# davidea97/Fisher-Nerf-customized

Hardware: AMD Instinct MI355X
Metric: candidate-views/sec (higher is better)
Workload: dtype f32

## Files before the change

### fisher-nerf-customized_amd/csrc/fisher_rast.hip

```cpp
#include <hip/hip_runtime.h>
#include <hip/hip_fp16.h>
#include <stdint.h>
#include <stdio.h>
#include <stdlib.h>
#include <string.h>
#include "fr_math.h"
#include "../../include/fisher_rast.h"
#include "fr_internal.h"

#define FR_THREADS 256
#define FR_G_MAX 32
#define FR_MAX_LDS_TILES 4096
#define FR_PART_MIN_DEFAULT 2048
#define FR_SORT_SMALL_KEYS 2048
#define FR_SORT_MID_KEYS 4096
#define FR_SORT_BIG_KEYS 16384
#define FR_VC_MAX 16
#define FR_BATCH 256
#define FR_BWD_BATCH 128

#include <vector>
#include <utility>
static thread_local char g_err[512] = "";
#if defined(FR_ABLATE) || defined(FR_LOOPSTATS)
// ... 474 lines not shown
	}
	constexpr int NB = 8;
	for (int g0 = 0; g0 < p.G; g0 += NB)
	{
		int rad[NB];
		float4 q0[NB];
		float dep[NB];
#pragma unroll
		for (int b = 0; b < NB; b++)
		{
			const int i = (blockIdx.x * p.G + g0 + b) * FR_THREADS + tid;
			rad[b] = (g0 + b < p.G && i < p.P) ? p.radii[vP + i] : 0;
		}
#pragma unroll
		for (int b = 0; b < NB; b++)
		{
			const int i = (blockIdx.x * p.G + g0 + b) * FR_THREADS + tid;
			if (rad[b] > 0)
			{
				const float4* sp = (const float4*)(p.splat + vP + i);
				q0[b] = sp[0];
				dep[b] = sp[1].z;
			}
		}
#pragma unroll
		for (int b = 0; b < NB; b++)
		{
			if (rad[b] > 0)
			{
				const int i = (blockIdx.x * p.G + g0 + b) * FR_THREADS + tid;
				const uint64_t hi = ((uint64_t)fr_as_u32(dep[b])) << 32;
				const fr_rect rc = fr_get_rect(q0[b].x, q0[b].y, rad[b], p.gx, p.gy);
				for (uint32_t y = rc.y0; y < rc.y1; y++)
					for (uint32_t x = rc.x0; x < rc.x1; x++)
					{
						const uint32_t t = y * p.gx + x;
						const uint32_t slot = lds ? (s_base[t] + atomicAdd(&s_cnt[t], 1u)) : (off[t] + atomicAdd(&fill[t], 1u));
						p.keys[slot] = hi | (uint32_t)i;
					}
			}
		}
	}
}

struct FrRecordArgs {
	const float* H_inv; long long hinv_stride; const float* packed; float4* recq;
	const float4* mt;
	const float4* grp;
	int early;
	float4* comp;
	uint32_t* slot_idx;
	int stride;
	float* slot_acc;
};
template <int C> struct FrPackSize { static constexpr int value = (C >= 11) ? 32 : 16; };
template <int C, bool REWRITE, bool FORM_A = false, bool FIVE = false, bool IDV = false>
__device__ __forceinline__ void fr_fisher_record_one(const FrParams& p, const float* __restrict__ H_inv, long long hinv_stride,
                                                     const float* __restrict__ packed, float4* __restrict__ recq, int v, uint32_t id,
                                                     const float* vm, const float* pm, const float* wm, bool has_w2c,
                                                     float4* out6 = nullptr, const float4* ab_src = nullptr);
template <int C, int AF, bool DK = false> struct FrRecStride { static constexpr int value = AF == 4 ? 3 : AF >= 2 ? (C >= 11 ? 13 : 7) : ((AF == 0 && DK) ? 5 : 6); };
template <int C, bool POSE = false>
__device__ __forceinline__ void fr_fisher_record_general(const FrParams& p, const float* __restrict__ packed, int v, uint32_t id,
                                                         const float* vm, const float* pm, const float* wm, bool has_w2c,
                                                         float4* out, const float4* ab_src);

template <int RC, bool PHASE_C>
__global__ __launch_bounds__(FR_THREADS) void k_preprocess_views(FrParams p, FrRecordArgs ra)
{
	extern __shared__ uint32_t fr_dyn_lds[];
	const int VC = p.VC;
	uint32_t* hist = fr_dyn_lds;
	uint32_t* pairs = hist + (size_t)VC * p.T;
	float* s_wm = (float*)(pairs + FR_THREADS * VC);
	const int W32 = 8 * p.G;
	uint32_t* s_bm = (uint32_t*)(s_wm + 12 * VC);
	uint32_t* s_pf = s_bm + VC * W32;
	const bool compact = RC != 0 && ra.comp != nullptr;
	__shared__ uint32_t s_np;
	__shared__ uint32_t s_n[FR_VC_MAX];
	__shared__ uint32_t s_ref[FR_VC_MAX];
	const int tid = threadIdx.x, lane = tid & 63;
	const int v0 = blockIdx.y * VC;
	const int nv = min(VC, p.V - v0);
	const uint32_t nblk = gridDim.x;
	const uint32_t cap = (uint32_t)(FR_THREADS * p.G);
	for (int t = tid; t < nv * p.T; t += FR_THREADS) hist[t] = 0;
	const bool has_w2c = p.w2c != nullptr;
	if (has_w2c) for (int t = tid; t < nv * 12; t += FR_THREADS) s_wm[t] = p.w2c[16 * (size_t)(v0 + t / 12) + (t % 12)];
	if (tid < FR_VC_MAX) { s_n[tid] = 0; s_ref[tid] = 0; }
	if (tid == 0) s_np = 0;
	if (compact) for (int t = tid; t < nv * W32; t += FR_THREADS) s_bm[t] = 0u;
	float vm[16], pm[16];
#pragma unroll
	for (int k = 0; k < 16; k++) { vm[k] = p.view[k]; pm[k] = p.proj[k]; }
	__syncthreads();
	for (int g = 0; g < p.G; g++)
	{
		const int i0 = (blockIdx.x * p.G + g) * FR_THREADS;
		if (i0 >= p.P) break;
		{
			const int i = i0 + tid;
			const bool live = i < p.P;
			fr_f3 pw = { 0.f, 0.f, 0.f };
			if (live) pw = fr_f3{ p.means3D[3 * (size_t)i], p.means3D[3 * (size_t)i + 1], p.means3D[3 * (size_t)i + 2] };
			const bool early = RC != 0 && ra.early != 0 && ra.mt != nullptr;
			float tr = 0.f;
// ... 137 lines not shown
		if (p.vis_count && s_n[tid]) atomicAdd(&p.vis_count[v], (int)s_n[tid]);
		if (p.num_rendered && s_ref[tid]) atomicAdd(&p.num_rendered[v], (int)s_ref[tid]);
	}
	if constexpr (RC != 0 && PHASE_C)
	{
		__syncthreads();
		if (compact)
		{
			for (int t = tid; t < nv * W32; t += FR_THREADS)
			{
				const int vv = t / W32, w = t - vv * W32;
				uint32_t acc = 0;
				for (int u = 0; u < w; u++) acc += (uint32_t)__popc(s_bm[vv * W32 + u]);
				s_pf[t] = acc;
			}
			__syncthreads();
		}
		const size_t PV = (size_t)nblk * cap;
		for (int vv = 0; vv < nv; vv++)
		{
			const int v = v0 + vv;
			const uint32_t n = s_n[vv];
			FrVisEntry* list = p.vis_list + ((size_t)v * nblk + blockIdx.x) * cap;
			float wm[12];
#pragma unroll
			for (int k = 0; k < 12; k++) wm[k] = has_w2c ? s_wm[12 * vv + k] : 0.f;
			for (uint32_t e = tid; e < n; e += FR_THREADS)
			{
				const uint32_t idx = list[e].idx;
				if (compact)
				{
					const uint32_t local = idx - blockIdx.x * cap;
					const uint32_t rank = s_pf[vv * W32 + (int)(local >> 5)] + (uint32_t)__popc(s_bm[vv * W32 + (int)(local >> 5)] & ((1u << (local & 31u)) - 1u));
					const uint32_t slot = blockIdx.x * cap + rank;
					const float4* tmp = (const float4*)(p.splat + ((size_t)v * nblk + blockIdx.x) * cap + e);
					fr_fisher_record_one<(RC < 0 ? -RC : RC), false, (RC < 0)>(p, ra.H_inv, ra.hinv_stride, ra.packed, ra.recq, v, idx, vm, pm, wm, has_w2c,
					                                                           ra.comp + ((size_t)v * PV + slot) * 6, tmp);
					list[e].idx = slot;
					if constexpr (RC < 0) ra.slot_idx[(size_t)v * PV + slot] = idx;
				}
				else fr_fisher_record_one<(RC < 0 ? -RC : RC), false, (RC < 0)>(p, ra.H_inv, ra.hinv_stride, ra.packed, ra.recq, v, idx, vm, pm, wm, has_w2c);
			}
		}
	}
}

template <int C, int AF, bool DK, bool IDV = false, bool SLOTS = false>
__global__ __launch_bounds__(FR_THREADS) void k_preprocess_views_c(FrParams p, FrRecordArgs ra)
{
	static_assert(!SLOTS || (AF == 0 && !IDV), "the slot table is an option of the general score form (the out_H forms always write it)");
	static_assert((C == 4 || C == 11) && AF >= 0 && AF <= 4 && !((AF == 1 || AF >= 3) && C != 4), "records modes: score form, A-form (4 columns), general out_H form, pose form (4 columns), render form (4 columns)");
	static_assert(!IDV || (C == 4 && AF == 0 && DK), "the identity-view front end is the 4-column score form's with fixed key segments");
	constexpr int RS = FrRecStride<C, AF, DK>::value;
	extern __shared__ uint32_t fr_dyn_lds[];
	const int VC = p.VC;
	uint32_t* hist = fr_dyn_lds;
	uint32_t* pairs = hist + (size_t)VC * p.T;
	float* s_wm = (float*)(pairs + FR_THREADS * (VC + 1));
	uint32_t* park = (uint32_t*)(s_wm + 12 * VC);
	__shared__ uint32_t s_n[FR_VC_MAX];
	__shared__ uint32_t s_ref[FR_VC_MAX];
	__shared__ uint32_t s_ca[FR_VC_MAX * 4];
	__shared__ uint32_t s_wk2[2][FR_VC_MAX * 4];
	__shared__ uint32_t s_wtot2[2][4];
	uint32_t batch_no = 0;
	const int tid = threadIdx.x, lane = tid & 63;
	const int wave = __builtin_amdgcn_readfirstlane(tid >> 6);
	const int v0 = blockIdx.y * VC;
	const int nv = min(VC, p.V - v0);
	const uint32_t nblk = gridDim.x;
	const uint32_t cap = (uint32_t)(FR_THREADS * p.G);
	for (int t = tid; t < nv * p.T; t += FR_THREADS) hist[t] = 0;
	const bool has_w2c = p.w2c != nullptr;
	if (has_w2c) for (int t = tid; t < nv * 12; t += FR_THREADS) s_wm[t] = p.w2c[16 * (size_t)(v0 + t / 12) + (t % 12)];
	if (tid < FR_VC_MAX) { s_n[tid] = 0; s_ref[tid] = 0; }
	float vm[16], pm[16];
#pragma unroll
	for (int k = 0; k < 16; k++) { vm[k] = IDV ? (k % 5 == 0 ? 1.f : 0.f) : p.view[k]; pm[k] = p.proj[k]; }
	if constexpr (IDV)
	{
		bool id = true;
#pragma unroll
		for (int k = 0; k < 16; k++) id = id && p.view[k] == vm[k];
		if (!id && tid == 0) { atomicOr(&p.status[1], 1); atomicOr(&p.status[3], 2); }
	}
	const size_t PV = (size_t)nblk * cap;
	const unsigned long long lt = (1ull << lane) - 1ull;
	__syncthreads();
	const int iw = blockIdx.x * p.G * FR_THREADS;
	const bool early = ra.early != 0;
	const float lx = 1.3f * p.tanfovx, ly = 1.3f * p.tanfovy;
	float wn;
	{
		const float c0 = fabsf(vm[0]) + fabsf(vm[1]) + fabsf(vm[2]), c1 = fabsf(vm[4]) + fabsf(vm[5]) + fabsf(vm[6]), c2 = fabsf(vm[8]) + fabsf(vm[9]) + fabsf(vm[10]);
		const float r0 = fabsf(vm[0]) + fabsf(vm[4]) + fabsf(vm[8]), r1 = fabsf(vm[1]) + fabsf(vm[5]) + fabsf(vm[9]), r2 = fabsf(vm[2]) + fabsf(vm[6]) + fabsf(vm[10]);
		wn = fmaxf(c0, fmaxf(c1, c2)) * fmaxf(r0, fmaxf(r1, r2));
	}
	const float fx2 = 1.02f * wn * p.focal_x * p.focal_x, fy2 = 1.02f * wn * p.focal_y * p.focal_y;
	const float xmax = (float)(p.gx * FR_BLOCK_X + FR_BLOCK_X), ymax = (float)(p.gy * FR_BLOCK_Y + FR_BLOCK_Y);
	unsigned long long skipm = 0ull;
	if (early && ra.grp != nullptr && p.G * nv <= 64)
	{
		const float wrow = fabsf(pm[3] - vm[2]) + fabsf(pm[7] - vm[6]) + fabsf(pm[11] - vm[10]) + fabsf(pm[15] - vm[14]);
		const float wmag = fabsf(vm[2]) + fabsf(vm[6]) + fabsf(vm[10]) + fabsf(vm[14]);
		const bool pinhole = wrow <= 1e-6f * wmag;
		bool skip = false;
		const int g = lane / nv, vv = lane - g * nv;
		const int blk = blockIdx.x * p.G + g;
		if (pinhole && g < p.G && blk * FR_THREADS < p.P)
		{
#pragma clang fp contract(fast)
			const float4 b0 = ra.grp[2 * (size_t)blk], b1 = ra.grp[2 * (size_t)blk + 1];
			const fr_f3 cw = { 0.5f * (b0.x + b1.x), 0.5f * (b0.y + b1.y), 0.5f * (b0.z + b1.z) };
			const float ex = b1.x - cw.x, ey = b1.y - cw.y, ez = b1.z - cw.z;
			float R = 1.01f * __builtin_amdgcn_sqrtf(ex * ex + ey * ey + ez * ez) + 1e-6f;
			const fr_f3 c = has_w2c ? fr_world_to_cam(cw, s_wm + 12 * vv) : cw;
			if (has_w2c)
			{
				const float* m = s_wm + 12 * vv;
				const float g00 = m[0] * m[0] + m[4] * m[4] + m[8] * m[8], g11 = m[1] * m[1] + m[5] * m[5] + m[9] * m[9], g22 = m[2] * m[2] + m[6] * m[6] + m[10] * m[10];
				const float g01 = fabsf(m[0] * m[1] + m[4] * m[5] + m[8] * m[9]), g02 = fabsf(m[0] * m[2] + m[4] * m[6] + m[8] * m[10]), g12 = fabsf(m[1] * m[2] + m[5] * m[6] + m[9] * m[10]);
				R *= __builtin_amdgcn_sqrtf(fmaxf(g00 + g01 + g02, fmaxf(g01 + g11 + g12, g02 + g12 + g22))) * 1.00001f;
			}
			const float kcm = fx2 * (1.0f + lx * lx) + fy2 * (1.0f + ly * ly);
			const float a2 = 2.0f * 1.01f * 3.0f * __builtin_amdgcn_sqrtf(kcm * b0.w);
			const float c0 = 6.0f;
			const float Wf = (float)p.W, Hf = (float)p.H;
			const float zc = vm[2] * c.x + vm[6] * c.y + vm[10] * c.z + vm[14];
			const float zn = __builtin_amdgcn_sqrtf(vm[2] * vm[2] + vm[6] * vm[6] + vm[10] * vm[10]);
			auto side = [&](float sx, float sy, float sz, float sw, float kz, float add) -> bool {
				const float Ax = sx + kz * vm[2], Ay = sy + kz * vm[6], Az = sz + kz * vm[10];
				const float Lc = Ax * c.x + Ay * c.y + Az * c.z + (sw + kz * vm[14]) + add;
				return Lc + __builtin_amdgcn_sqrtf(Ax * Ax + Ay * Ay + Az * Az) * R < 0.f;
			};
			const bool left = side(Wf * pm[0], Wf * pm[4], Wf * pm[8], Wf * pm[12], Wf - 1.0f + 2.0f * c0, a2);
			const bool right = side(-Wf * pm[0], -Wf * pm[4], -Wf * pm[8], -Wf * pm[12], -(Wf - 1.0f - 2.0f * xmax - 2.0f * c0), a2);
			const bool top = side(Hf * pm[1], Hf * pm[5], Hf * pm[9], Hf * pm[13], Hf - 1.0f + 2.0f * c0, a2);
			const bool bottom = side(-Hf * pm[1], -Hf * pm[5], -Hf * pm[9], -Hf * pm[13], -(Hf - 1.0f - 2.0f * ymax - 2.0f * c0), a2);
			const bool behind = zc + zn * R <= 0.001f;
			skip = left || right || top || bottom || behind;
		}
		skipm = __builtin_amdgcn_ballot_w64(skip);
	}
	uint32_t pend = 0;
	for (int g = 0; g < p.G; g++)
	{
		const int i0 = iw + g * FR_THREADS;
		if (i0 >= p.P) break;
		const bool last_round = g == p.G - 1 || i0 + FR_THREADS >= p.P;
		uint32_t np = 0;
		const uint32_t skipv = (uint32_t)(skipm >> (g * nv)) & ((1u << nv) - 1u);
		if (skipv != (1u << nv) - 1u)
		{
			const int i = i0 + tid;
			const bool live = i < p.P;
			fr_f3 pw = { 0.f, 0.f, 0.f };
			float tr = 0.f;
			if (live) { const float4 m4 = ra.mt[i]; pw = fr_f3{ m4.x, m4.y, m4.z }; tr = m4.w; }
			uint32_t keepbits = 0;
			for (int vv = 0; vv < nv; vv++)
			{
// ... 128 lines not shown
					{
						const int tx0 = (int)ceilf((sp.px - hx - 15.0f) * 0.0625f), sy0 = (int)ceilf((sp.py - hy - 3.0f) * 0.25f);
						const int sy1 = (int)floorf((sp.py + hy) * 0.25f) + 1;
						rx0 = (uint32_t)max((int)rx0, tx0); rx1 = max(rx0, rx1);
						ry0 = (uint32_t)max((int)ry0, sy0); ry1 = (uint32_t)max((int)ry0, min((int)ry1, sy1));
					}
					if (rx1 > rx0 && ry1 > ry0)
						for (uint32_t y = ry0 >> 2; y <= (ry1 - 1u) >> 2; y++)
							for (uint32_t x = rx0; x < rx1; x++)
								atomicAdd(&h[y * p.gx + x], 1u);
				}
				else
				for (uint32_t y = ry0; y < ry1; y++)
					for (uint32_t x = rx0; x < rx1; x++)
						atomicAdd(&h[y * p.gx + x], 1u);
				park[0 * FR_THREADS + pos] = __float_as_uint(sp.px);
				park[1 * FR_THREADS + pos] = __float_as_uint(sp.py);
				park[2 * FR_THREADS + pos] = ext;
				if constexpr (AF == 4)
				{
					park[3 * FR_THREADS + pos] = __float_as_uint(o);
					park[4 * FR_THREADS + pos] = __float_as_uint(sp.conx);
					park[5 * FR_THREADS + pos] = __float_as_uint(sp.cony);
					park[6 * FR_THREADS + pos] = __float_as_uint(sp.conz);
				}
				else
				{
					park[3 * FR_THREADS + pos] = __float_as_uint(__builtin_amdgcn_logf(o));
					park[4 * FR_THREADS + pos] = __float_as_uint(-0.5f * sp.conx);
					park[5 * FR_THREADS + pos] = __float_as_uint(-sp.cony);
					park[6 * FR_THREADS + pos] = __float_as_uint(-0.5f * sp.conz);
				}
				park[7 * FR_THREADS + pos] = __float_as_uint(cg);
				park[8 * FR_THREADS + pos] = (uint32_t)i;
				park[9 * FR_THREADS + pos] = fr_as_u32(sp.depth);
				park[10 * FR_THREADS + pos] = rx0 | (ry0 << 16);
				park[11 * FR_THREADS + pos] = rx1 | (ry1 << 16);
				park[12 * FR_THREADS + pos] = rank | ((uint32_t)vv << 16);
			}
			__syncthreads();
			if (tid < nv) s_n[tid] += (s_wk[tid * 4] + s_wk[tid * 4 + 1]) + (s_wk[tid * 4 + 2] + s_wk[tid * 4 + 3]);
			FR_ABL(if (p.ablate == 36) nvis = 0;)
			if ((uint32_t)tid < nvis)
			{
					const int r = tid;
				float4 ab[2];
				ab[0] = make_float4(__uint_as_float(park[0 * FR_THREADS + r]), __uint_as_float(park[1 * FR_THREADS + r]),
				                    __uint_as_float(park[2 * FR_THREADS + r]), __uint_as_float(park[3 * FR_THREADS + r]));
				ab[1] = make_float4(__uint_as_float(park[4 * FR_THREADS + r]), __uint_as_float(park[5 * FR_THREADS + r]),
				                    __uint_as_float(park[6 * FR_THREADS + r]), __uint_as_float(park[7 * FR_THREADS + r]));
				const uint32_t idx = park[8 * FR_THREADS + r];
				const uint32_t rk = park[12 * FR_THREADS + r];
				const int cvv = (int)(rk >> 16);
				const uint32_t slot = blockIdx.x * cap + (rk & 0xffffu);
				const int v = v0 + cvv;
				float wm[12];
#pragma unroll
				for (int k = 0; k < 12; k++) wm[k] = has_w2c ? s_wm[12 * cvv + k] : 0.f;
				float4* rec_out = ra.comp + ((size_t)v * PV + slot) * RS;
				FR_ABL(if (p.ablate == 37) rec_out = ra.comp + (size_t)tid * RS;)
				if constexpr (AF == 4)
				{
					const float4 t2 = ((const float4*)(ra.packed + (size_t)idx * FrPackSize<C>::value))[2];
					rec_out[0] = ab[0];
					rec_out[1] = make_float4(ab[1].x, ab[1].y, ab[1].z, __uint_as_float(park[9 * FR_THREADS + r]));
					rec_out[2] = make_float4(t2.y, t2.z, t2.w, ab[1].w);
				}
				else if constexpr (AF >= 2) fr_fisher_record_general<C, (AF == 3)>(p, ra.packed, v, idx, vm, pm, wm, has_w2c, rec_out, ab);
				else fr_fisher_record_one<C, false, (AF == 1), (AF == 0 && DK), IDV>(p, ra.H_inv, ra.hinv_stride, ra.packed, ra.recq, v, idx, vm, pm, wm, has_w2c, rec_out, ab);
				if constexpr (DK)
				{
					const uint32_t xy0 = park[10 * FR_THREADS + r], xy1 = park[11 * FR_THREADS + r];
					const uint32_t rect = (xy0 & 255u) | ((xy0 >> 16) << 8) | (((xy1 & 0xffffu) - (xy0 & 0xffffu)) << 16) | (((xy1 >> 16) - (xy0 >> 16)) << 24);
					((uint2*)p.vis_list)[((size_t)v * nblk + blockIdx.x) * cap + (rk & 0xffffu)] = make_uint2(park[9 * FR_THREADS + r], rect);
				}
				else
				{
					FrVisEntry en;
					en.idx = slot; en.depth_bits = park[9 * FR_THREADS + r];
					en.xy0 = park[10 * FR_THREADS + r]; en.xy1 = park[11 * FR_THREADS + r];
					*(uint4*)(p.vis_list + ((size_t)v * nblk + blockIdx.x) * cap + (rk & 0xffffu)) = *(const uint4*)&en;
				}
				if constexpr (AF == 1 || AF == 2 || SLOTS) ra.slot_idx[(size_t)v * PV + slot] = p.order ? p.order[idx] : idx;
				if constexpr (SLOTS) ra.slot_acc[(size_t)v * PV + slot] = 0.f;
			}
		}
		const uint32_t rem = pend - ndo;
		if (rem != 0u && ndo != 0u)
		{
			uint32_t t = 0;
			if ((uint32_t)tid < rem) t = pairs[ndo + tid];
			__syncthreads();
			if ((uint32_t)tid < rem) pairs[tid] = t;
			__syncthreads();
		}
		pend = rem;
	}
	__syncthreads();
	if constexpr (DK)
	{
		uint32_t* cursor = park + 13 * FR_THREADS;
		uint32_t vend[FR_VC_MAX];
		uint32_t ntot = 0;
#pragma unroll
		for (int k = 0; k < FR_VC_MAX; k++) { if (k < nv) ntot += s_n[k]; vend[k] = ntot; }
		FR_ABL(if (p.ablate == 31) ntot = 0;)
		constexpr int NB = 4;
		uint2 en[NB], nx[NB];
		uint32_t ev[NB], nxv[NB];
		auto load_round = [&](uint32_t e0, uint2 (&de)[NB], uint32_t (&dv)[NB])
		{
#pragma unroll
			for (int b = 0; b < NB; b++)
			{
				const uint32_t e = e0 + b * FR_THREADS + tid;
				uint32_t vv = 0, lo = 0;
#pragma unroll
				for (int k = 0; k < FR_VC_MAX - 1; k++) if (e >= vend[k]) { vv = k + 1; lo = vend[k]; }
				dv[b] = vv;
				de[b] = make_uint2(0u, 0u);
				FR_ABL(if (p.ablate == 33) { if (e < ntot) de[b] = make_uint2(e, (e & 7u) | ((e >> 3 & 15u) << 10) | (2u << 16) | (2u << 24)); } else)
				if (e < ntot) de[b] = ((const uint2*)p.vis_list)[((size_t)(v0 + vv) * nblk + blockIdx.x) * cap + (e - lo)];
			}
		};
		load_round(0u, en, ev);
		const int nb = nv * p.T;
		for (int b0 = 0; b0 < nb; b0 += 4 * FR_THREADS)
		{
			uint32_t c[4], at[4], gt[4];
#pragma unroll
			for (int k = 0; k < 4; k++)
			{
				const int b = b0 + k * FR_THREADS + tid;
				c[k] = b < nb ? hist[b] : 0u;
				gt[k] = (uint32_t)(v0 + b / p.T) * (uint32_t)p.T + (uint32_t)(b % p.T);
			}
#pragma unroll
			for (int k = 0; k < 4; k++)
			{
				at[k] = 0u;
				FR_ABL(if (p.ablate != 34))
				if (c[k]) at[k] = atomicAdd(&p.tile_cnt[gt[k]], c[k]);
			}
#pragma unroll
			for (int k = 0; k < 4; k++)
			{
				const int b = b0 + k * FR_THREADS + tid;
				if (b < nb)
				{
					hist[b] = (c[k] && at[k] + c[k] <= p.tile_cap) ? gt[k] * p.tile_cap + at[k] : 0xffffffffu;
					cursor[b] = 0u;
				}
			}
		}
		__syncthreads();
		for (uint32_t e0 = 0; e0 < ntot; e0 += NB * FR_THREADS)
		{
			const bool more = e0 + NB * FR_THREADS < ntot;
			if (more) load_round(e0 + NB * FR_THREADS, nx, nxv);
#pragma unroll
			for (int b = 0; b < NB; b++)
			{
				const uint32_t e = e0 + b * FR_THREADS + tid;
				const uint32_t lo = ev[b] ? vend[ev[b] - 1] : 0u;
				const uint64_t key = ((uint64_t)en[b].x << 32) | ((blockIdx.x * cap + (e - lo)) << 4);
				const uint32_t r = en[b].y;
				const uint32_t x0 = r & 255u, s0 = (r >> 8) & 255u, x1 = x0 + ((r >> 16) & 255u), s1 = s0 + (r >> 24);
				const uint32_t* hb = hist + (size_t)ev[b] * p.T;
				uint32_t* cu = cursor + (size_t)ev[b] * p.T;
				if (x1 > x0 && s1 > s0)
				for (uint32_t y = s0 >> 2; y <= (s1 - 1u) >> 2; y++)
				{
					const uint32_t a = max(s0, 4u * y) - 4u * y, z = min(s1, 4u * y + 4u) - 4u * y;
					const uint64_t ky = key | (uint64_t)(((1u << z) - 1u) & ~((1u << a) - 1u));
					for (uint32_t x = x0; x < x1; x++)
					{
						const uint32_t t = y * p.gx + x;
						const uint32_t base = hb[t];
						const uint32_t k = atomicAdd(&cu[t], 1u);
						FR_ABL(if (p.ablate != 32 && p.ablate != 33))
						if (base != 0xffffffffu) p.keys[base + k] = ky;
					}
				}
			}
			if (more)
			{
#pragma unroll
				for (int b = 0; b < NB; b++) { en[b] = nx[b]; ev[b] = nxv[b]; }
			}
		}
	}
	else
	{
		for (int vv = 0; vv < nv; vv++)
		{
			const int v = v0 + vv;
			uint32_t* cnt = p.tile_cnt + (size_t)v * p.T;
			const uint32_t* h = hist + (size_t)vv * p.T;
			for (int t = tid; t < p.T; t += FR_THREADS)
			{
				const uint32_t c = h[t];
				if (c) p.blk_base[((size_t)v * nblk + blockIdx.x) * p.T + t] = atomicAdd(&cnt[t], c);
			}
		}
	}
	if (tid < nv)
	{
		const int v = v0 + tid;
		p.vis_n[(size_t)v * nblk + blockIdx.x] = s_n[tid];
		if (p.vis_count && s_n[tid]) atomicAdd(&p.vis_count[v], (int)s_n[tid]);
		if (p.num_rendered && s_ref[tid]) atomicAdd(&p.num_rendered[v], (int)s_ref[tid]);
	}
}
__global__ __launch_bounds__(FR_THREADS) void k_scatter_vis(FrParams p)
{
	extern __shared__ uint32_t fr_dyn_lds[];
	uint32_t* s_cnt = fr_dyn_lds;
	uint32_t* s_base = fr_dyn_lds + p.T;
	if (p.status[1]) return;
	const int tid = threadIdx.x;
	const int v = blockIdx.y;
	const uint32_t nblk = gridDim.x;
	const uint32_t n = p.vis_n[(size_t)v * nblk + blockIdx.x];
	if (n == 0) return;
	const uint32_t* off = p.tile_off + (size_t)v * p.T;
	const uint32_t* bb = p.blk_base + ((size_t)v * nblk + blockIdx.x) * p.T;
	for (int t = tid; t < p.T; t += FR_THREADS) { s_cnt[t] = 0; s_base[t] = off[t] + bb[t]; }
	__syncthreads();
	const uint4* list = (const uint4*)(p.vis_list + ((size_t)v * nblk + blockIdx.x) * (size_t)(FR_THREADS * p.G));
	constexpr int NB = 4;
	for (uint32_t e0 = 0; e0 < n; e0 += NB * FR_THREADS)
	{
		uint4 en[NB];
#pragma unroll
		for (int b = 0; b < NB; b++)
		{
			const uint32_t e = e0 + b * FR_THREADS + tid;
			en[b] = e < n ? list[e] : make_uint4(0u, 0u, 0u, 0u);
		}
#pragma unroll
		for (int b = 0; b < NB; b++)
		{
			const uint64_t key = ((uint64_t)en[b].y << 32) | en[b].x;
			const uint32_t x0 = en[b].z & 0xffffu, y0 = en[b].z >> 16, x1 = en[b].w & 0xffffu, y1 = en[b].w >> 16;
			for (uint32_t y = y0; y < y1; y++)
				for (uint32_t x = x0; x < x1; x++)
				{
					const uint32_t t = y * p.gx + x;
					p.keys[s_base[t] + atomicAdd(&s_cnt[t], 1u)] = key;
				}
		}
	}
}

__device__ __forceinline__ void fr_tile_of_block(const FrParams& p, uint32_t& tile, int& v, uint32_t first = 0u)
{
	const uint32_t L = blockIdx.x - first;
	if ((p.V & 7) == 0)
	{
		const uint32_t xcd = L & 7u, q = L >> 3;
		v = (int)((q / (uint32_t)p.T) * 8u + xcd);
		if (p.view_perm) v = (int)p.view_perm[v];
		tile = q % (uint32_t)p.T;
	}
	else
	{
		v = (int)(L / (uint32_t)p.T);
		tile = L % (uint32_t)p.T;
	}
}

__device__ __forceinline__ void fr_cx(uint64_t& lo, uint64_t& hi)
{
	const uint64_t a = lo, b = hi;
	const bool sw = a > b;
	lo = sw ? b : a; hi = sw ? a : b;
}
template <typename KeyPtr>
__device__ __forceinline__ uint64_t fr_ldk(KeyPtr keys, uint32_t i, uint32_t n) { return i < n ? keys[i] : ~0ull; }
template <typename KeyPtr>
__device__ __forceinline__ void fr_stk(KeyPtr keys, uint32_t i, uint32_t n, uint64_t v) { if (i < n) keys[i] = v; }

template <typename KeyPtr>
__device__ __forceinline__ void fr_bitonic(KeyPtr keys, uint32_t n, int tid, const uint32_t FR_NT = FR_THREADS)
{
	uint32_t n_pad = 1;
	while (n_pad < n) n_pad <<= 1;
	if (n_pad < 2) return;
	for (uint32_t t = tid; t < (n_pad >> 1); t += FR_NT)
	{
		uint64_t a = fr_ldk(keys, 2 * t, n), b = fr_ldk(keys, 2 * t + 1, n);
		fr_cx(a, b);
		fr_stk(keys, 2 * t, n, a); fr_stk(keys, 2 * t + 1, n, b);
	}
	__syncthreads();
	const uint32_t groups = n_pad >> 2;
	for (uint32_t k = 4, lk = 2; k <= n_pad; k <<= 1, lk++)
	{
		{
			const uint32_t q = k >> 2, qm = q - 1u;
			for (uint32_t g = tid; g < groups; g += FR_NT)
			{
				const uint32_t base = (g >> (lk - 2)) << lk, r = g & qm;
				const uint32_t ia = base + r, ib = ia + q, id = base + k - 1u - r, ic = id - q;
				uint64_t a = fr_ldk(keys, ia, n), b = fr_ldk(keys, ib, n), c = fr_ldk(keys, ic, n), d = fr_ldk(keys, id, n);
				fr_cx(a, d); fr_cx(b, c);
				fr_cx(a, b); fr_cx(c, d);
				fr_stk(keys, ia, n, a); fr_stk(keys, ib, n, b); fr_stk(keys, ic, n, c); fr_stk(keys, id, n, d);
			}
			__syncthreads();
		}
		uint32_t j = k >> 3, lj = lk - 3;
		for (; j >= 2; j >>= 2, lj -= 2)
		{
			const uint32_t h = j >> 1, lh = lj - 1, hm = h - 1u;
			for (uint32_t g = tid; g < groups; g += FR_NT)
			{
				const uint32_t i0 = ((g >> lh) << (lh + 2)) + (g & hm);
				const uint32_t i1 = i0 + h, i2 = i0 + j, i3 = i2 + h;
				uint64_t a = fr_ldk(keys, i0, n), b = fr_ldk(keys, i1, n), c = fr_ldk(keys, i2, n), d = fr_ldk(keys, i3, n);
				fr_cx(a, c); fr_cx(b, d);
				fr_cx(a, b); fr_cx(c, d);
// ... 5110 lines not shown
struct FrScorerPlan { int columns; bool form_a; FrRecordArgs ra; bool skip_pack = false; bool general = false; bool pose = false; bool view_identity = false; bool render = false; bool point = false; };
template <int C> __global__ void k_pack_static(FrParams p, const float* __restrict__ H_inv, float* __restrict__ packed, float4* __restrict__ mt, float4* __restrict__ grp);
template <int C, bool LIST, bool FORM_A> __global__ void k_fisher_records(FrParams p, FrRecordArgs ra);

static int fr_bin_pipeline(FrParams& p, const fr_gaussians* g, hipStream_t s, const FrScorerPlan* plan = nullptr)
{
	int rc;
	const int P = p.P;
	{
		FrZeroer z;
		z.add(p.tile_cnt, (size_t)p.V * p.T * 4); z.add(p.status, 16); z.add(p.big_list, 64);
		if (p.part_list) z.add(p.part_list, 4);
		if (p.view_work) z.add(p.view_work, (size_t)p.V * 4);
		if (p.vis_count) z.add(p.vis_count, (size_t)p.V * 4);
		if (p.num_rendered && p.vis_list != nullptr && p.T <= FR_MAX_LDS_TILES) z.add(p.num_rendered, (size_t)p.V * 4);
		z.launch(s);
	}
	const bool multi = p.vis_list != nullptr && p.T <= FR_MAX_LDS_TILES;
	if (g->cov3D_precomp) p.cov3D = g->cov3D_precomp;
	else if (plan && multi) p.cov3D = nullptr;
	else
	{
		hipLaunchKernelGGL(k_cov3d, dim3((P + FR_THREADS - 1) / FR_THREADS), dim3(FR_THREADS), 0, s, P, g->scales, p.mod, g->rotations, p.cov3D_out);
		if ((rc = fr_check_launch("k_cov3d"))) return rc;
		p.cov3D = p.cov3D_out;
	}
	p.G = multi ? fr_pick_G_views(P) : fr_pick_G(P, p.V);
	p.VC = fr_pick_VC(p.T);
	const int per_block = FR_THREADS * p.G;
	dim3 gridP((P + per_block - 1) / per_block, p.V);
	const size_t hist_lds = p.T <= FR_MAX_LDS_TILES ? (size_t)p.T * 4 : 16;
	if (plan && !plan->skip_pack)
	{
		const float* shared_hinv = plan->ra.hinv_stride ? nullptr : plan->ra.H_inv;
		dim3 gp((P + FR_THREADS - 1) / FR_THREADS);
		if (plan->columns == 4) hipLaunchKernelGGL((k_pack_static<4>), gp, dim3(FR_THREADS), 0, s, p, shared_hinv, (float*)plan->ra.packed, (float4*)plan->ra.mt, (float4*)plan->ra.grp);
		else hipLaunchKernelGGL((k_pack_static<11>), gp, dim3(FR_THREADS), 0, s, p, shared_hinv, (float*)plan->ra.packed, (float4*)plan->ra.mt, (float4*)plan->ra.grp);
		if ((rc = fr_check_launch("k_pack_static"))) return rc;
	}
	FrJoinGuard joins(s);
	if (multi)
	{
		const bool once = plan && plan->ra.comp != nullptr && fr_debug_mode() != 20;
		if (!once) p.tile_cap = 0;
		const bool wanted_fixed = p.tile_cap != 0;
		if (once) p.VC = fr_plan_views_c(p.T, p.VC, p.tile_cap);
		if (once && wanted_fixed && !p.tile_cap) return fr_fail(FR_EINVAL, "fr_bin_pipeline: fixed key segments planned, but they do not fit the LDS");
		auto lds_c_of = [&](int vc) { return fr_lds_views_c(vc, p.T, p.tile_cap != 0); };
		dim3 gridV(gridP.x, (p.V + p.VC - 1) / p.VC);
		const size_t lds = ((size_t)p.VC * p.T + (size_t)FR_THREADS * p.VC + 12 * (size_t)p.VC + 2 * (size_t)p.VC * 8 * (size_t)p.G) * 4;
		FrRecordArgs ra = plan ? plan->ra : FrRecordArgs{ nullptr, 0, nullptr, nullptr, nullptr, nullptr, 0, nullptr, nullptr, 6 };
		const bool dk = p.tile_cap != 0;
		const size_t lds_c = lds_c_of(p.VC);
		if (once && plan->render && dk) hipLaunchKernelGGL((k_preprocess_views_c<4, 4, true>), gridV, dim3(FR_THREADS), lds_c, s, p, ra);
		else if (once && plan->render) hipLaunchKernelGGL((k_preprocess_views_c<4, 4, false>), gridV, dim3(FR_THREADS), lds_c, s, p, ra);
		else if (once && plan->pose && dk) hipLaunchKernelGGL((k_preprocess_views_c<4, 3, true>), gridV, dim3(FR_THREADS), lds_c, s, p, ra);
		else if (once && plan->pose) hipLaunchKernelGGL((k_preprocess_views_c<4, 3, false>), gridV, dim3(FR_THREADS), lds_c, s, p, ra);
		else if (once && plan->general && plan->columns == 4 && dk) hipLaunchKernelGGL((k_preprocess_views_c<4, 2, true>), gridV, dim3(FR_THREADS), lds_c, s, p, ra);
		else if (once && plan->general && plan->columns == 4) hipLaunchKernelGGL((k_preprocess_views_c<4, 2, false>), gridV, dim3(FR_THREADS), lds_c, s, p, ra);
		else if (once && plan->general && dk) hipLaunchKernelGGL((k_preprocess_views_c<11, 2, true>), gridV, dim3(FR_THREADS), lds_c, s, p, ra);
		else if (once && plan->general) hipLaunchKernelGGL((k_preprocess_views_c<11, 2, false>), gridV, dim3(FR_THREADS), lds_c, s, p, ra);
		else if (once && plan->form_a && dk) hipLaunchKernelGGL((k_preprocess_views_c<4, 1, true>), gridV, dim3(FR_THREADS), lds_c, s, p, ra);
		else if (once && plan->form_a) hipLaunchKernelGGL((k_preprocess_views_c<4, 1, false>), gridV, dim3(FR_THREADS), lds_c, s, p, ra);
		else if (once && plan->point && plan->columns == 4 && dk) hipLaunchKernelGGL((k_preprocess_views_c<4, 0, true, false, true>), gridV, dim3(FR_THREADS), lds_c, s, p, ra);
		else if (once && plan->point && plan->columns == 4) hipLaunchKernelGGL((k_preprocess_views_c<4, 0, false, false, true>), gridV, dim3(FR_THREADS), lds_c, s, p, ra);
		else if (once && plan->point && dk) hipLaunchKernelGGL((k_preprocess_views_c<11, 0, true, false, true>), gridV, dim3(FR_THREADS), lds_c, s, p, ra);
		else if (once && plan->point) hipLaunchKernelGGL((k_preprocess_views_c<11, 0, false, false, true>), gridV, dim3(FR_THREADS), lds_c, s, p, ra);
		else if (once && plan->columns == 4 && dk && plan->view_identity) hipLaunchKernelGGL((k_preprocess_views_c<4, 0, true, true>), gridV, dim3(FR_THREADS), lds_c, s, p, ra);
		else if (once && plan->columns == 4 && dk) hipLaunchKernelGGL((k_preprocess_views_c<4, 0, true>), gridV, dim3(FR_THREADS), lds_c, s, p, ra);
		else if (once && plan->columns == 4) hipLaunchKernelGGL((k_preprocess_views_c<4, 0, false>), gridV, dim3(FR_THREADS), lds_c, s, p, ra);
		else if (once && dk) hipLaunchKernelGGL((k_preprocess_views_c<11, 0, true>), gridV, dim3(FR_THREADS), lds_c, s, p, ra);
		else if (once) hipLaunchKernelGGL((k_preprocess_views_c<11, 0, false>), gridV, dim3(FR_THREADS), lds_c, s, p, ra);
		else if (!plan) hipLaunchKernelGGL((k_preprocess_views<0, false>), gridV, dim3(FR_THREADS), lds, s, p, ra);
#ifdef FR_AB
		else if (plan->form_a) hipLaunchKernelGGL((k_preprocess_views<-4, true>), gridV, dim3(FR_THREADS), lds, s, p, ra);
		else if (plan->columns == 4) hipLaunchKernelGGL((k_preprocess_views<4, true>), gridV, dim3(FR_THREADS), lds, s, p, ra);
		else hipLaunchKernelGGL((k_preprocess_views<11, true>), gridV, dim3(FR_THREADS), lds, s, p, ra);
#else
		else return fr_fail(FR_EINVAL, "fr_bin_pipeline: a records plan of the multi-view front end needs compact records");
#endif
		if ((rc = fr_check_launch("k_preprocess_views"))) return rc;
	}
	else
	{
		p.tile_cap = 0;
		hipLaunchKernelGGL(k_preprocess, gridP, dim3(FR_THREADS), hist_lds, s, p);
		if ((rc = fr_check_launch("k_preprocess"))) return rc;
	}
	if (multi && p.tile_cap >= 2u * (uint32_t)FR_SORT_SMALL_KEYS + 128u && fr_debug_mode() != 32)
	{
		p.small_max = (uint32_t)FR_PART_MIN_DEFAULT;
		FR_AB_ONLY({ const int e = fr_env_int("FR_PART_MIN"); if (e >= 512 && e <= FR_SORT_SMALL_KEYS) p.small_max = (uint32_t)e; })
	}
	if (multi && p.tile_cap)
		hipLaunchKernelGGL(k_tile_lists, dim3((p.V * p.T + 4 * FR_THREADS - 1) / (4 * FR_THREADS)), dim3(FR_THREADS), 0, s, p.tile_cnt, p.tile_off, p.V * p.T, p.T,
		                   p.tile_cap, p.status, p.big_list, p.view_work, p.view_perm, p.ablate, p.small_max);
	else
	hipLaunchKernelGGL(k_scan_tiles, dim3(1), dim3(1024), 0, s, p.tile_cnt, p.tile_off, p.tile_fill, p.V * p.T, p.T, p.V,
	                   p.key_capacity, p.status, multi ? (int*)nullptr : p.num_rendered, p.big_list, p.view_work, p.view_perm);
	if ((rc = fr_check_launch("k_scan_tiles"))) return rc;
	if (multi && p.tile_cap) {  }
	else if (multi) hipLaunchKernelGGL(k_scatter_vis, gridP, dim3(FR_THREADS), 2 * hist_lds, s, p);
	else hipLaunchKernelGGL(k_scatter_keys, gridP, dim3(FR_THREADS), 2 * hist_lds, s, p);
	if ((rc = fr_check_launch("k_scatter_keys"))) return rc;
	if (plan && !multi)
	{
		FrSideStream& s2 = fr_side_stream(1);
		const bool forked2 = s2.ok && hipEventRecord(s2.fork, s) == hipSuccess && hipStreamWaitEvent(s2.stream, s2.fork, 0) == hipSuccess;
		hipStream_t rs = forked2 ? s2.stream : s;
		if (plan->form_a) hipLaunchKernelGGL((k_fisher_records<4, false, true>), gridP, dim3(FR_THREADS), 0, rs, p, plan->ra);
		else if (plan->columns == 4) hipLaunchKernelGGL((k_fisher_records<4, false, false>), gridP, dim3(FR_THREADS), 0, rs, p, plan->ra);
		else hipLaunchKernelGGL((k_fisher_records<11, false, false>), gridP, dim3(FR_THREADS), 0, rs, p, plan->ra);
		if (forked2) joins.forked(&s2);
		if ((rc = fr_check_launch("k_fisher_records"))) return rc;
	}
	FrSideStream& side = fr_side_stream();
	const bool part_all = p.tile_cap >= 32768u && fr_debug_mode() != 32;
	const bool want_fork = fr_debug_mode() != 7 && (!multi || p.V >= 8) && !part_all;
	const bool forked = want_fork && side.ok && hipEventRecord(side.fork, s) == hipSuccess && hipStreamWaitEvent(side.stream, side.fork, 0) == hipSuccess;
	const int big_blocks = p.T * p.V < 256 ? p.T * p.V : 256;
	if (forked) joins.forked(&side);
	uint32_t part_max = 0;
	if (p.part_list && p.tile_cap >= 2u * (uint32_t)FR_SORT_SMALL_KEYS + 128u && fr_debug_mode() != 32)
	{
		part_max = p.tile_cap / 2u - 64u;
// ... 1661 lines not shown
```

Before: 47980.

## Remap preprocess workgroups into grouped (block, view-chunk) order for locality

Replaces the 2D grid of the compact multi-view preprocess kernel with a 1D grid. A device helper decodes each workgroup ID into a Gaussian block and a view chunk, grouping runs of 8 blocks by view-chunk groups (CG). The aim is to make concurrently scheduled workgroups share Gaussian and view data in cache, or to spread them across XCDs. With the default CG equal to the number of chunks, this is block-major ordering in groups of 8. The change adds per-block index math and a padded grid where out-of-range workgroups return early.

```diff
diff --git a/fisher-nerf-customized_amd/csrc/fisher_rast.hip b/fisher-nerf-customized_amd/csrc/fisher_rast.hip
--- a/fisher-nerf-customized_amd/csrc/fisher_rast.hip
+++ b/fisher-nerf-customized_amd/csrc/fisher_rast.hip
@@ -550,7 +550,9 @@
 	uint32_t* slot_idx;
 	int stride;
 	float* slot_acc;
+	int NB, NC, CG;
 };
+__device__ __forceinline__ bool fr_fe_block(const FrRecordArgs& ra, uint32_t& blk, uint32_t& chunk);
 template <int C> struct FrPackSize { static constexpr int value = (C >= 11) ? 32 : 16; };
 template <int C, bool REWRITE, bool FORM_A = false, bool FIVE = false, bool IDV = false>
 __device__ __forceinline__ void fr_fisher_record_one(const FrParams& p, const float* __restrict__ H_inv, long long hinv_stride,
@@ -794,6 +796,8 @@
 	static_assert((C == 4 || C == 11) && AF >= 0 && AF <= 4 && !((AF == 1 || AF >= 3) && C != 4), "records modes: score form, A-form (4 columns), general out_H form, pose form (4 columns), render form (4 columns)");
 	static_assert(!IDV || (C == 4 && AF == 0 && DK), "the identity-view front end is the 4-column score form's with fixed key segments");
 	constexpr int RS = FrRecStride<C, AF, DK>::value;
+	uint32_t bx, cy;
+	if (!fr_fe_block(ra, bx, cy)) return;
 	extern __shared__ uint32_t fr_dyn_lds[];
 	const int VC = p.VC;
 	uint32_t* hist = fr_dyn_lds;
@@ -808,9 +812,9 @@
 	uint32_t batch_no = 0;
 	const int tid = threadIdx.x, lane = tid & 63;
 	const int wave = __builtin_amdgcn_readfirstlane(tid >> 6);
-	const int v0 = blockIdx.y * VC;
+	const int v0 = (int)cy * VC;
 	const int nv = min(VC, p.V - v0);
-	const uint32_t nblk = gridDim.x;
+	const uint32_t nblk = (uint32_t)ra.NB;
 	const uint32_t cap = (uint32_t)(FR_THREADS * p.G);
 	for (int t = tid; t < nv * p.T; t += FR_THREADS) hist[t] = 0;
 	const bool has_w2c = p.w2c != nullptr;
@@ -829,7 +833,7 @@
 	const size_t PV = (size_t)nblk * cap;
 	const unsigned long long lt = (1ull << lane) - 1ull;
 	__syncthreads();
-	const int iw = blockIdx.x * p.G * FR_THREADS;
+	const int iw = bx * p.G * FR_THREADS;
 	const bool early = ra.early != 0;
 	const float lx = 1.3f * p.tanfovx, ly = 1.3f * p.tanfovy;
 	float wn;
@@ -848,7 +852,7 @@
 		const bool pinhole = wrow <= 1e-6f * wmag;
 		bool skip = false;
 		const int g = lane / nv, vv = lane - g * nv;
-		const int blk = blockIdx.x * p.G + g;
+		const int blk = bx * p.G + g;
 		if (pinhole && g < p.G && blk * FR_THREADS < p.P)
 		{
 #pragma clang fp contract(fast)
@@ -1083,7 +1087,7 @@
 				const uint32_t idx = park[8 * FR_THREADS + r];
 				const uint32_t rk = park[12 * FR_THREADS + r];
 				const int cvv = (int)(rk >> 16);
-				const uint32_t slot = blockIdx.x * cap + (rk & 0xffffu);
+				const uint32_t slot = bx * cap + (rk & 0xffffu);
 				const int v = v0 + cvv;
 				float wm[12];
 #pragma unroll
@@ -1103,14 +1107,14 @@
 				{
 					const uint32_t xy0 = park[10 * FR_THREADS + r], xy1 = park[11 * FR_THREADS + r];
 					const uint32_t rect = (xy0 & 255u) | ((xy0 >> 16) << 8) | (((xy1 & 0xffffu) - (xy0 & 0xffffu)) << 16) | (((xy1 >> 16) - (xy0 >> 16)) << 24);
-					((uint2*)p.vis_list)[((size_t)v * nblk + blockIdx.x) * cap + (rk & 0xffffu)] = make_uint2(park[9 * FR_THREADS + r], rect);
+					((uint2*)p.vis_list)[((size_t)v * nblk + bx) * cap + (rk & 0xffffu)] = make_uint2(park[9 * FR_THREADS + r], rect);
 				}
 				else
 				{
 					FrVisEntry en;
 					en.idx = slot; en.depth_bits = park[9 * FR_THREADS + r];
 					en.xy0 = park[10 * FR_THREADS + r]; en.xy1 = park[11 * FR_THREADS + r];
-					*(uint4*)(p.vis_list + ((size_t)v * nblk + blockIdx.x) * cap + (rk & 0xffffu)) = *(const uint4*)&en;
+					*(uint4*)(p.vis_list + ((size_t)v * nblk + bx) * cap + (rk & 0xffffu)) = *(const uint4*)&en;
 				}
 				if constexpr (AF == 1 || AF == 2 || SLOTS) ra.slot_idx[(size_t)v * PV + slot] = p.order ? p.order[idx] : idx;
 				if constexpr (SLOTS) ra.slot_acc[(size_t)v * PV + slot] = 0.f;
@@ -1151,7 +1155,7 @@
 				dv[b] = vv;
 				de[b] = make_uint2(0u, 0u);
 				FR_ABL(if (p.ablate == 33) { if (e < ntot) de[b] = make_uint2(e, (e & 7u) | ((e >> 3 & 15u) << 10) | (2u << 16) | (2u << 24)); } else)
-				if (e < ntot) de[b] = ((const uint2*)p.vis_list)[((size_t)(v0 + vv) * nblk + blockIdx.x) * cap + (e - lo)];
+				if (e < ntot) de[b] = ((const uint2*)p.vis_list)[((size_t)(v0 + vv) * nblk + bx) * cap + (e - lo)];
 			}
 		};
 		load_round(0u, en, ev);
@@ -1194,7 +1198,7 @@
 			{
 				const uint32_t e = e0 + b * FR_THREADS + tid;
 				const uint32_t lo = ev[b] ? vend[ev[b] - 1] : 0u;
-				const uint64_t key = ((uint64_t)en[b].x << 32) | ((blockIdx.x * cap + (e - lo)) << 4);
+				const uint64_t key = ((uint64_t)en[b].x << 32) | ((bx * cap + (e - lo)) << 4);
 				const uint32_t r = en[b].y;
 				const uint32_t x0 = r & 255u, s0 = (r >> 8) & 255u, x1 = x0 + ((r >> 16) & 255u), s1 = s0 + (r >> 24);
 				const uint32_t* hb = hist + (size_t)ev[b] * p.T;
@@ -1231,14 +1235,14 @@
 			for (int t = tid; t < p.T; t += FR_THREADS)
 			{
 				const uint32_t c = h[t];
-				if (c) p.blk_base[((size_t)v * nblk + blockIdx.x) * p.T + t] = atomicAdd(&cnt[t], c);
+				if (c) p.blk_base[((size_t)v * nblk + bx) * p.T + t] = atomicAdd(&cnt[t], c);
 			}
 		}
 	}
 	if (tid < nv)
 	{
 		const int v = v0 + tid;
-		p.vis_n[(size_t)v * nblk + blockIdx.x] = s_n[tid];
+		p.vis_n[(size_t)v * nblk + bx] = s_n[tid];
 		if (p.vis_count && s_n[tid]) atomicAdd(&p.vis_count[v], (int)s_n[tid]);
 		if (p.num_rendered && s_ref[tid]) atomicAdd(&p.num_rendered[v], (int)s_ref[tid]);
 	}
@@ -1299,6 +1303,19 @@
 		v = (int)(L / (uint32_t)p.T);
 		tile = L % (uint32_t)p.T;
 	}
+}
+
+__device__ __forceinline__ bool fr_fe_block(const FrRecordArgs& ra, uint32_t& blk, uint32_t& chunk)
+{
+	FR_AB_ONLY(if (ra.CG == 0) { blk = blockIdx.x; chunk = blockIdx.y; return true; })
+	const uint32_t L = blockIdx.x, x = L & 7u, q = L >> 3;
+	const uint32_t NB = (uint32_t)ra.NB, NC = (uint32_t)ra.NC, CG = (uint32_t)ra.CG;
+	const uint32_t per = ((NB + 7u) >> 3) * CG;
+	const uint32_t gq = q / per, r = q - gq * per;
+	const uint32_t j = r / CG;
+	blk = (uint32_t)__builtin_amdgcn_readfirstlane((int)(j * 8u + x));
+	chunk = (uint32_t)__builtin_amdgcn_readfirstlane((int)(gq * CG + (r - j * CG)));
+	return blk < NB && chunk < NC;
 }
 
 __device__ __forceinline__ void fr_cx(uint64_t& lo, uint64_t& hi)
@@ -6515,25 +6532,36 @@
 		FrRecordArgs ra = plan ? plan->ra : FrRecordArgs{ nullptr, 0, nullptr, nullptr, nullptr, nullptr, 0, nullptr, nullptr, 6 };
 		const bool dk = p.tile_cap != 0;
 		const size_t lds_c = lds_c_of(p.VC);
-		if (once && plan->render && dk) hipLaunchKernelGGL((k_preprocess_views_c<4, 4, true>), gridV, dim3(FR_THREADS), lds_c, s, p, ra);
-		else if (once && plan->render) hipLaunchKernelGGL((k_preprocess_views_c<4, 4, false>), gridV, dim3(FR_THREADS), lds_c, s, p, ra);
-		else if (once && plan->pose && dk) hipLaunchKernelGGL((k_preprocess_views_c<4, 3, true>), gridV, dim3(FR_THREADS), lds_c, s, p, ra);
-		else if (once && plan->pose) hipLaunchKernelGGL((k_preprocess_views_c<4, 3, false>), gridV, dim3(FR_THREADS), lds_c, s, p, ra);
-		else if (once && plan->general && plan->columns == 4 && dk) hipLaunchKernelGGL((k_preprocess_views_c<4, 2, true>), gridV, dim3(FR_THREADS), lds_c, s, p, ra);
-		else if (once && plan->general && plan->columns == 4) hipLaunchKernelGGL((k_preprocess_views_c<4, 2, false>), gridV, dim3(FR_THREADS), lds_c, s, p, ra);
-		else if (once && plan->general && dk) hipLaunchKernelGGL((k_preprocess_views_c<11, 2, true>), gridV, dim3(FR_THREADS), lds_c, s, p, ra);
-		else if (once && plan->general) hipLaunchKernelGGL((k_preprocess_views_c<11, 2, false>), gridV, dim3(FR_THREADS), lds_c, s, p, ra);
-		else if (once && plan->form_a && dk) hipLaunchKernelGGL((k_preprocess_views_c<4, 1, true>), gridV, dim3(FR_THREADS), lds_c, s, p, ra);
-		else if (once && plan->form_a) hipLaunchKernelGGL((k_preprocess_views_c<4, 1, false>), gridV, dim3(FR_THREADS), lds_c, s, p, ra);
-		else if (once && plan->point && plan->columns == 4 && dk) hipLaunchKernelGGL((k_preprocess_views_c<4, 0, true, false, true>), gridV, dim3(FR_THREADS), lds_c, s, p, ra);
-		else if (once && plan->point && plan->columns == 4) hipLaunchKernelGGL((k_preprocess_views_c<4, 0, false, false, true>), gridV, dim3(FR_THREADS), lds_c, s, p, ra);
-		else if (once && plan->point && dk) hipLaunchKernelGGL((k_preprocess_views_c<11, 0, true, false, true>), gridV, dim3(FR_THREADS), lds_c, s, p, ra);
-		else if (once && plan->point) hipLaunchKernelGGL((k_preprocess_views_c<11, 0, false, false, true>), gridV, dim3(FR_THREADS), lds_c, s, p, ra);
-		else if (once && plan->columns == 4 && dk && plan->view_identity) hipLaunchKernelGGL((k_preprocess_views_c<4, 0, true, true>), gridV, dim3(FR_THREADS), lds_c, s, p, ra);
-		else if (once && plan->columns == 4 && dk) hipLaunchKernelGGL((k_preprocess_views_c<4, 0, true>), gridV, dim3(FR_THREADS), lds_c, s, p, ra);
-		else if (once && plan->columns == 4) hipLaunchKernelGGL((k_preprocess_views_c<4, 0, false>), gridV, dim3(FR_THREADS), lds_c, s, p, ra);
-		else if (once && dk) hipLaunchKernelGGL((k_preprocess_views_c<11, 0, true>), gridV, dim3(FR_THREADS), lds_c, s, p, ra);
-		else if (once) hipLaunchKernelGGL((k_preprocess_views_c<11, 0, false>), gridV, dim3(FR_THREADS), lds_c, s, p, ra);
+		ra.NB = (int)gridV.x; ra.NC = (int)gridV.y; ra.CG = ra.NC;
+#ifdef FR_AB
+		{
+			static const bool given = getenv("FR_FE_CG") != nullptr;
+			static const int forced = fr_env_int("FR_FE_CG");
+			if (given) ra.CG = forced < 0 ? 0 : (forced > ra.NC ? ra.NC : forced);
+		}
+#endif
+		const unsigned long long nwg = ra.CG ? 8ull * ((gridV.x + 7u) / 8u) * (unsigned)ra.CG * (unsigned)((ra.NC + ra.CG - 1) / ra.CG) : 0ull;
+		if (once && nwg > 0x7fffffffull) return fr_fail(FR_EINVAL, "fr_bin_pipeline: too many (Gaussian block, view chunk) workgroups for one launch");
+		const dim3 gridC = ra.CG ? dim3((uint32_t)nwg) : gridV;
+		if (once && plan->render && dk) hipLaunchKernelGGL((k_preprocess_views_c<4, 4, true>), gridC, dim3(FR_THREADS), lds_c, s, p, ra);
+		else if (once && plan->render) hipLaunchKernelGGL((k_preprocess_views_c<4, 4, false>), gridC, dim3(FR_THREADS), lds_c, s, p, ra);
+		else if (once && plan->pose && dk) hipLaunchKernelGGL((k_preprocess_views_c<4, 3, true>), gridC, dim3(FR_THREADS), lds_c, s, p, ra);
+		else if (once && plan->pose) hipLaunchKernelGGL((k_preprocess_views_c<4, 3, false>), gridC, dim3(FR_THREADS), lds_c, s, p, ra);
+		else if (once && plan->general && plan->columns == 4 && dk) hipLaunchKernelGGL((k_preprocess_views_c<4, 2, true>), gridC, dim3(FR_THREADS), lds_c, s, p, ra);
+		else if (once && plan->general && plan->columns == 4) hipLaunchKernelGGL((k_preprocess_views_c<4, 2, false>), gridC, dim3(FR_THREADS), lds_c, s, p, ra);
+		else if (once && plan->general && dk) hipLaunchKernelGGL((k_preprocess_views_c<11, 2, true>), gridC, dim3(FR_THREADS), lds_c, s, p, ra);
+		else if (once && plan->general) hipLaunchKernelGGL((k_preprocess_views_c<11, 2, false>), gridC, dim3(FR_THREADS), lds_c, s, p, ra);
+		else if (once && plan->form_a && dk) hipLaunchKernelGGL((k_preprocess_views_c<4, 1, true>), gridC, dim3(FR_THREADS), lds_c, s, p, ra);
+		else if (once && plan->form_a) hipLaunchKernelGGL((k_preprocess_views_c<4, 1, false>), gridC, dim3(FR_THREADS), lds_c, s, p, ra);
+		else if (once && plan->point && plan->columns == 4 && dk) hipLaunchKernelGGL((k_preprocess_views_c<4, 0, true, false, true>), gridC, dim3(FR_THREADS), lds_c, s, p, ra);
+		else if (once && plan->point && plan->columns == 4) hipLaunchKernelGGL((k_preprocess_views_c<4, 0, false, false, true>), gridC, dim3(FR_THREADS), lds_c, s, p, ra);
+		else if (once && plan->point && dk) hipLaunchKernelGGL((k_preprocess_views_c<11, 0, true, false, true>), gridC, dim3(FR_THREADS), lds_c, s, p, ra);
+		else if (once && plan->point) hipLaunchKernelGGL((k_preprocess_views_c<11, 0, false, false, true>), gridC, dim3(FR_THREADS), lds_c, s, p, ra);
+		else if (once && plan->columns == 4 && dk && plan->view_identity) hipLaunchKernelGGL((k_preprocess_views_c<4, 0, true, true>), gridC, dim3(FR_THREADS), lds_c, s, p, ra);
+		else if (once && plan->columns == 4 && dk) hipLaunchKernelGGL((k_preprocess_views_c<4, 0, true>), gridC, dim3(FR_THREADS), lds_c, s, p, ra);
+		else if (once && plan->columns == 4) hipLaunchKernelGGL((k_preprocess_views_c<4, 0, false>), gridC, dim3(FR_THREADS), lds_c, s, p, ra);
+		else if (once && dk) hipLaunchKernelGGL((k_preprocess_views_c<11, 0, true>), gridC, dim3(FR_THREADS), lds_c, s, p, ra);
+		else if (once) hipLaunchKernelGGL((k_preprocess_views_c<11, 0, false>), gridC, dim3(FR_THREADS), lds_c, s, p, ra);
 		else if (!plan) hipLaunchKernelGGL((k_preprocess_views<0, false>), gridV, dim3(FR_THREADS), lds, s, p, ra);
 #ifdef FR_AB
 		else if (plan->form_a) hipLaunchKernelGGL((k_preprocess_views<-4, true>), gridV, dim3(FR_THREADS), lds, s, p, ra);
```

Measured after the change: 48330, median of 6. About the same (+0.7%).
